# Totoketchup/Adaptive-MultiSpeaker-Separation

Measured on AMD Instinct MI355X. Metric: mixtures/sec training throughput (2-spk, 256-filter adapt+BLSTM-DPCL), higher is better.
Workload: dtype f32 (storage, accumulation and results f32; dense products issued on the 16-bit matrix pipe as fp16x3 / bf16x6 emulation of the f32 product -- `value_native_f32` is the same step on v_mfma_f32_32x32x2_f32)

## Files before the change

### adaptive-multispeaker-separation_amd/ams_hip/functional.py

```python
import torch
from torch.autograd import Function

from . import ops


def _c(t):
    return t if t.is_contiguous() else t.contiguous()


class _Overlap(object):

    def __init__(self):
        self.enabled = False
        self.stream = None
        self.n_cap = 0
        self.deferred = []
        self.on_ready = None

    def side(self):
        if self.stream is None:
            import os
            self.stream = torch.cuda.Stream(priority=int(os.environ.get('AMS_SIDE_PRIORITY', '0')))
        return self.stream

# ... 29 lines not shown
            def __enter__(self_):
                ov.cap(True, kind)

            def __exit__(self_, *exc):
                ov.cap(False)
        return _Cap()

    def ready(self, *params):
        if self.on_ready is not None:
            self.on_ready(params, self.side())

    def defer(self, fn):
        self.deferred.append(fn)

    def flush(self, n=1):
        s = self.side()
        with torch.cuda.stream(s):
            for _ in range(min(n, len(self.deferred))):
                self.deferred.pop(0)()

    def join(self):
        if self.deferred:
            s = self.side()
            s.wait_stream(torch.cuda.current_stream())
            self.flush(len(self.deferred))
        self.n_cap = 0
        if self.stream is not None:
            torch.cuda.current_stream().wait_stream(self.stream)


OVERLAP = _Overlap()


class FrontFilter(Function):

    @staticmethod
    def forward(ctx, w, bases):
        ctx.save_for_backward(w, bases)
        return ops.front_filter(w, bases)

    @staticmethod
    def backward(ctx, df):
        w, bases = ctx.saved_tensors
        return ops.front_filter_bwd(w, bases, _c(df))


class FrontConv(Function):

    @staticmethod
    def forward(ctx, x, f, hop):
        ctx.save_for_backward(x)
        ctx.W, ctx.hop = f.shape[0], hop
        am = (ops.amax_of(x), ops.amax_of(f)) if (ops.F16X3 and x.is_cuda) else None
        return ops.front_conv(x, f, hop, amax=am, measure=True)

    @staticmethod
    def backward(ctx, dy):
        (x,) = ctx.saved_tensors
        df = ops.front_conv_bwd_filter(x, _c(dy), ctx.W, ctx.hop) if ctx.needs_input_grad[1] else None
        return None, df, None


import os as _os
_DW_SPLIT = [int(v) for v in _os.environ.get('AMS_DW_SPLIT', '24,12,4').split(',') if v]


def _dw_cuts(N):
    tiles = N // 256
    if N % 256 or len(_DW_SPLIT) < 2 or tiles < sum(_DW_SPLIT):
        return [(0, N)]
    tot = sum(_DW_SPLIT)
    cuts, n0 = [], 0
    for i, f in enumerate(_DW_SPLIT):
        n1 = N if i == len(_DW_SPLIT) - 1 else n0 + (tiles * f // tot) * 256
        if n1 > n0:
            cuts.append((n0, n1))
        n0 = n1
    return cuts

class BLSTMLayer(Function):

    @staticmethod
    def forward(ctx, x, Kf, bf, Kb, bb, last_capped=False):
        aw = ops.param_amax(Kf) if ops.F16X3 and x.is_cuda else None
        if aw is not None and aw is not ops.param_amax(Kb):
            aw = None
        ax = ops.amax_of(x) if aw is not None else None
        ctx.amax = (ax, aw) if aw is not None else None
        out, G, cst = ops.blstm_fwd(x, Kf, bf, Kb, bb, amax=ctx.amax)
        if x.is_cuda:
            ops.tag_amax(out, ops.amax_one(out.device))
        ctx.last_capped = bool(last_capped)
        ctx.save_for_backward(x, Kf, Kb, out, G, cst)
        ctx.biases = (bf, bb)
        return out

    @staticmethod
    def backward(ctx, dout):
        x, Kf, Kb, out, G, cst = ctx.saved_tensors
        bf, bb = ctx.biases
        need_dx = ctx.needs_input_grad[0]
        if OVERLAP.usable(Kf, Kb, bf, bb) and all(ctx.needs_input_grad[1:5]):
            B, T, D = x.shape
            dbpart = ops.blstm_bwd_recurrent(x, Kf, Kb, G, cst, _c(dout), amax_u=ctx.amax[1] if ctx.amax is not None else None)
            am_dx = am_w = None
            if ctx.amax is not None:
                az = ops.amax_of(G)
                am_dx = (az, ctx.amax[1])
                am_w = (ctx.amax[0], ops.amax_one(G.device), az)
            dx = ops.blstm_bwd_dx(G, Kf, Kb, B, T, D, amax=am_dx) if need_dx else None
            if not need_dx and ops.WGRAD_GROUP >= 1:
                ops.blstm_bwd_weights(x, out, G, Kf.grad, bf.grad, Kb.grad, bb.grad, True, part='all', dbpart=dbpart, amax=am_w)
                return None, None, None, None, None, None
            s = OVERLAP.fork(x, out, G, *([dbpart] if dbpart is not None else []))
            if not need_dx:
                with torch.cuda.stream(s):
                    ops.blstm_bwd_weights(x, out, G, Kf.grad, bf.grad, Kb.grad, bb.grad, True, part='u', amax=am_w)
                ops.blstm_bwd_weights(x, out, G, Kf.grad, bf.grad, Kb.grad, bb.grad, True, part='wx', dbpart=dbpart, amax=am_w)
                return None, None, None, None, None, None
            with torch.cuda.stream(s):
                with OVERLAP.capped('lstm'):
                    ops.blstm_bwd_weights(x, out, G, Kf.grad, bf.grad, Kb.grad, bb.grad, True, part='wx', dbpart=dbpart, amax=am_w)
# ... 10 lines not shown
class BLSTMLayerDropout(Function):

    @staticmethod
    def forward(ctx, x, Kf, bf, Kb, bb, m_in, m_h, m_c, m_out):
        masks = {'in': m_in, 'h': m_h, 'c': m_c, 'out': m_out}
        y, saved = ops.blstm_fwd_dropout(x, Kf, bf, Kb, bb, masks)
        ctx.save_for_backward(x, Kf, Kb, m_in, m_h, m_c, m_out, *saved)
        return y

    @staticmethod
    def backward(ctx, dy):
        x, Kf, Kb, m_in, m_h, m_c, m_out = ctx.saved_tensors[:7]
        saved = ctx.saved_tensors[7:]
        masks = {'in': m_in, 'h': m_h, 'c': m_c, 'out': m_out}
        dx, dKf, dbf, dKb, dbb = ops.blstm_bwd_dropout(_c(dy), x, Kf, Kb, saved, masks, need_dx=ctx.needs_input_grad[0])
        return dx, dKf, dbf, dKb, dbb, None, None, None, None


def blstm_dropout(x, Kf, bf, Kb, bb, keep, masks=None):
    if masks is None:
        B, T, D = x.shape
        masks = ops.blstm_dropout_masks(B, T, D, Kf.shape[1] // 4, keep, x.device)
    return BLSTMLayerDropout.apply(_c(x), Kf, bf, Kb, bb, masks['in'], masks['h'], masks['c'], masks['out'])


class Dense(Function):

    @staticmethod
    def forward(ctx, x, W, b):
        ctx.save_for_backward(x, W)
        ctx.bias = b
        aw = ops.param_amax(W) if ops.F16X3 and x.is_cuda else None
        ctx.amax = (ops.amax_of(x), aw) if aw is not None else None
        return ops.dense_fwd(x, W, b, amax=ctx.amax)

    @staticmethod
    def backward(ctx, du):
        x, W = ctx.saved_tensors
        du2 = _c(du).view(-1, W.shape[1])
        x2 = x.reshape(-1, x.shape[-1])
        b = ctx.bias
        am_dx = am_dw = None
        if ctx.amax is not None:
            adu = ops.amax_of(du2)
            am_dx, am_dw = (adu, ctx.amax[1]), (ctx.amax[0], adu)
        if OVERLAP.usable(W, b) and ctx.needs_input_grad[1] and ctx.needs_input_grad[2]:
            dx = ops.backward_product(du2, W, am_dx, (W,)).view(x.shape) if ctx.needs_input_grad[0] else None
            s = OVERLAP.fork(x2, du2)
            Nw = W.shape[1]
            cuts = _dw_cuts(Nw) if (ctx.needs_input_grad[0] and W.grad.stride(0) == Nw) else [(0, Nw)]

            def piece(n0, n1):
                Wg = W.grad if (n0, n1) == (0, Nw) else W.grad[:, n0:n1]
                dus = du2 if (n0, n1) == (0, Nw) else du2[:, n0:n1]
                with OVERLAP.capped('dense'):
                    fused = ops.gemm_at_b_colsum(x2, dus, Wg, b.grad[n0:n1], accumulate=True, amax=am_dw, ldc=W.grad.stride(0))
                    if not fused:
                        ops.gemm(x2, dus, transA=True, out=Wg, accumulate=True, amax=am_dw, M=x2.shape[1], N=n1 - n0, K=x2.shape[0],
                                 lda=x2.stride(0), ldb=du2.stride(0), ldc=W.grad.stride(0))
                if not fused:
                    ops.colsum_into(_c(dus), b.grad[n0:n1], True)
            with torch.cuda.stream(s):
                piece(*cuts[0])
            for i, c in enumerate(cuts[1:]):
                last = i == len(cuts) - 2
                OVERLAP.defer(lambda c=c, last=last: (piece(*c), OVERLAP.ready(W, b) if last else None))
# ... 766 lines not shown
```

### adaptive-multispeaker-separation_amd/ams_hip/ops.py

```python
import ctypes
import os as _os

import torch

from ._lib import load, check, AmsError

_vp = ctypes.c_void_p


def _p(t):
    return _vp(t.data_ptr()) if t is not None else _vp(0)


def _s():
    return _vp(torch.cuda.current_stream().cuda_stream)


def _chk(*ts):
    for t in ts:
        if t is None:
            continue
        if not t.is_cuda:
            raise AmsError('ams_hip ops need device tensors (there is no CPU fallback)')
        if t.dtype != torch.float32 or not t.is_contiguous():
# ... 664 lines not shown
        raise AmsError('ps_pack_cols: fp32 device matrix with dense rows expected')
    lib = load()
    K, N = w2.shape
    pitch = lib.ams_ps_image_pitch(K)
    if img is None:
        img = torch.empty((N, pitch), dtype=torch.uint8, device=w2.device)
    check(lib.ams_ps_pack_cols(_p(w2), w2.stride(0), _p(img), K, N, _p(amax), _s()), 'ams_ps_pack_cols')
    return img


def gemm_ps(a_img, b_img, K, amax, bias=None, out=None, ldc=None, label=''):
    lib = load()
    M, N = a_img.shape[0], b_img.shape[0]
    if out is None:
        out = torch.empty((M, N), dtype=torch.float32, device=a_img.device)
        ldc = N
    elif ldc is None:
        ldc = out.stride(0) if out.dim() == 2 else N
    ev = PROFILE.begin() if PROFILE.enabled else None
    cur = torch.cuda.current_stream()
    amax[0].record_stream(cur)
    amax[1].record_stream(cur)
    check(lib.ams_gemm_ps(M, N, K, _p(a_img), _p(b_img), _p(out), ldc, _p(bias), _p(amax[0]), _p(amax[1]), _s()), 'ams_gemm_ps')
    PS_LAUNCHES[0] += 1
    if ev is not None:
        PROFILE.end(ev, 2.0 * M * N * K, 4.0 * (M * K + K * N + M * N), 'gemm16ps<0,1>', label)
    return out


def _ps_weight_image(W2, amax_w, owners):
    return derived(owners, 'ps_w', lambda old: (ps_pack_cols(W2, amax_w), amax_w), key=(W2.data_ptr(), W2.shape, id(amax_w)))[0]


def forward_product_presplit(M, N, K, out, bias, amax, label, ldc):
    key = ('gemm', label, M, N, K, False, False)
    return (PRESPLIT and amax is not None and amax[0] is not None and amax[1] is not None and key not in F16_AUDIT.denied
            and not F16_AUDIT.active and LDS_PAD[0] == 0 and N % 4 == 0 and ldc % 4 == 0 and out.data_ptr() % 16 == 0
            and (bias is None or bias.data_ptr() % 16 == 0) and max(M, N) * ((K + 31) // 32 * 128) < 2 ** 31
            and load().ams_gemm_get_arith() != 0)


def forward_product(x2, W2, bias, out, amax, label, owners, ldc=None):
    M, K = x2.shape
    N = W2.shape[1]
    if x2.stride(1) != 1 or W2.stride(1) != 1:
        raise AmsError('forward_product: operands with dense rows expected (strides %r, %r)' % (tuple(x2.stride()), tuple(W2.stride())))
    ldc = (out.stride(0) if out.dim() == 2 else N) if ldc is None else ldc
    if not forward_product_presplit(M, N, K, out, bias, amax, label, ldc):
        return gemm(x2, W2, bias=bias, out=out, M=M, N=N, K=K, lda=x2.stride(0), ldb=W2.stride(0), ldc=ldc, label=label, amax=amax)
    a_img = ps_pack_rows(x2, amax[0])
    b_img = _ps_weight_image(W2, amax[1], owners)
    return gemm_ps(a_img, b_img, K, amax, bias=bias, out=out, ldc=ldc, label=label)


DX_PS = _os.environ.get('AMS_GEMM_DX_PS', '1') != '0'


def _ps_dx_weight_image(W2, amax_w, owners):
    return derived(owners, 'ps_dx', lambda old: (ps_pack_rows(W2, amax_w), amax_w), key=(W2.data_ptr(), W2.shape, id(amax_w)))[0]


def backward_product(dU2, W2, amax, owners, out=None, label=''):
    M, K = dU2.shape
    N = W2.shape[0]
    if out is None:
        out = torch.empty((M, N), dtype=torch.float32, device=dU2.device)
    ldc = out.stride(0) if out.dim() == 2 else N
    lda = dU2.stride(0)
    key = ('gemm', label, M, N, K, False, True)
    lib = load()
    if not (DX_PS and F16X3 and amax is not None and amax[0] is not None and amax[1] is not None and key not in F16_AUDIT.denied
            and not F16_AUDIT.active and LDS_PAD[0] == 0 and N % 4 == 0 and ldc % 4 == 0 and lda % 4 == 0 and dU2.stride(1) == 1
            and W2.stride(1) == 1 and out.data_ptr() % 16 == 0 and dU2.data_ptr() % 16 == 0 and M * lda * 4 < 2 ** 31
            and N * ((K + 31) // 32 * 128) < 2 ** 31 and lib.ams_gemm_get_arith() != 0
            and K % 4 == 0 and (N + 255) // 256 * 256 <= 1.30 * N):
        return gemm(dU2, W2, transB=True, out=out, M=M, N=N, K=K, lda=lda, ldb=W2.stride(0), ldc=ldc, label=label, amax=amax)
    b_img = _ps_dx_weight_image(W2, amax[1], owners)
    nb = lib.ams_gemm_ps_a_workspace_bytes(M, N, K)
    ws = _ws(nb, dU2) if nb else None
    ev = PROFILE.begin() if PROFILE.enabled else None
    cur = torch.cuda.current_stream()
    amax[0].record_stream(cur)
    amax[1].record_stream(cur)
    check(lib.ams_gemm_ps_a_f32(M, N, K, _p(dU2), lda, _p(b_img), _p(out), ldc, _p(amax[0]), _p(amax[1]), _p(ws), nb, _s()),
          'ams_gemm_ps_a_f32')
    if ev is not None:
        PROFILE.end(ev, 2.0 * M * N * K, 4.0 * (M * K + K * N + M * N), 'gemm16ps_a<0,1>', label)
    return out


def gemm_at_b_colsum(A, B, out, bsum, accumulate=True, amax=None, ldc=None):
    K, M = A.shape
    N = B.shape[1]
    ldc = out.stride(0) if ldc is None else ldc
    ok = (M % 4 == 0 and N % 4 == 0 and A.stride(0) % 4 == 0 and B.stride(0) % 4 == 0 and A.stride(1) == 1 and B.stride(1) == 1
          and out.stride(-1) == 1 and bsum.stride(-1) == 1 and not NOVEC)
    if not ok:
        return False
    if any(t.data_ptr() % 16 for t in (A, B, bsum)):
        gemm(A, B, transA=True, out=out, accumulate=accumulate, M=M, N=N, K=K, lda=A.stride(0), ldb=B.stride(0), ldc=ldc, amax=amax,
             key=('at_b_colsum', M, N, K))
        colsum_into(B if B.is_contiguous() else B.contiguous(), bsum, accumulate)
        return True
    lib = load()
    pad = LDS_PAD[0]
    nb = lib.ams_gemm_workspace_bytes(M, N, K, 1, pad)
    ws = _ws(nb, A) if nb else None
    bws = _ws(32 * N * 4, A)
# ... 79 lines not shown
def _err_words():
    live = [r for r in _ERR_EXTRA if r() is not None]
    _ERR_EXTRA[:] = live
    return list(_RING_ERR.values()) + [r() for r in live]


def ring_error_pending():
    return any(bool(t.item() != 0) for t in _err_words())


def ring_errors_clear():
    for t in _err_words():
        t.zero_()


def persist_errors():
    return int(ring_error_pending())


def raise_on_ring_errors():
    if ring_error_pending():
        ring_errors_clear()
        raise AmsError('a BLSTM ring recurrence launch abandoned a bounded wait: its workgroups were not all resident in time '
                       '(another kernel filled the CUs); the results of that step are invalid.  AMS_LSTM_RING=0 selects the '
                       'per-step recurrence kernels, which need no co-residency.')


def _padded_rows(x2, Dp):
    xp = torch.zeros((x2.shape[0], Dp), dtype=x2.dtype, device=x2.device)
    xp[:, :x2.shape[1]].copy_(x2)
    return xp


def blstm_fwd(x, Kf, bf, Kb, bb, amax=None):
    _chk(x, bf, bb)
    _chk_rows(Kf, Kb)
    lib = load()
    B, T, D = x.shape
    H = Kf.shape[1] // 4
    ldu = Kf.stride(0)
    if Kb.stride(0) != ldu:
        raise AmsError('blstm: the two direction kernels must share one row stride')
    x2 = x.view(B * T, D)
    frozen = _frozen(Kf, Kb, bf, bb)
    Wcat = derived((Kf, Kb), 'wcat', lambda old: blstm_wcat(Kf, Kb, D), key=(D,), keep='frozen')
    u_amax = amax[1] if amax is not None else None
    if amax is None and F16X3 and x.is_cuda:
        if frozen:
            u_amax = derived((Kf, Kb), 'kbound', lambda old: torch.maximum(absmax(Kf), absmax(Kb)), keep='frozen')
            amax = (amax_of(x), u_amax)
        else:
            amax = (amax_of(x), derived((Kf, Kb), 'wcat_amax', lambda old: absmax(Wcat, out=old)))
    if _twin(bf, bb):
        bias = torch.as_strided(bf, (8 * H,), (1,))
    else:
        bias = derived((bf, bb), 'bcat', lambda old: torch.cat([bf, bb]), keep='frozen')
    G = torch.empty((B, T, 2, 4 * H), dtype=torch.float32, device=x.device)
    nring = lib.ams_blstm_ring_sync_bytes(B, H, 0) if LSTM_RING != '0' else 0
    out = torch.empty((B, T, 2 * H), dtype=torch.float32, device=x.device)
    cst = torch.empty(((2, B, T, 2, H) if nring else (B, T, 2, H)), dtype=torch.float32, device=x.device)
    blstm_input_projection(x2, Wcat, bias, G.view(B * T, 8 * H), amax, (Kf, Kb))
    if nring:
        sync, pre0 = _ring_sync(nring, x)
        check(lib.ams_blstm_ring_fwd(_p(G), _p(out), _p(cst[0]), _p(cst[1]), _p(Kf[D:]), _p(Kb[D:]), ldu,
                                     _p(u_amax if F16X3 else None), _p(sync), nring, _p(ring_error_word(x.device)), B, T, H,
                                     int(LSTM_RING == 'safe') | pre0, _s()), 'ams_blstm_ring_fwd')
        return out, G, cst
    pack = torch.empty(lib.ams_blstm_pack_floats(H, 0), dtype=torch.float32, device=x.device)
    check(lib.ams_blstm_recurrent_fwd(_p(G), _p(out), _p(cst), _p(Kf[D:]), _p(Kb[D:]), ldu, _p(pack), B, T, H, _s()),
          'ams_blstm_recurrent_fwd')
    return out, G, cst


def blstm_input_projection(x2, Wcat, bias, G2, amax, owners):
    M, D = x2.shape
    N = Wcat.shape[1]
    label = 'blstm_input_gemm'
    Dp = (D + 3) // 4 * 4
    if Dp != D and not forward_product_presplit(M, N, D, G2, bias, amax, label, N):
        Wp = torch.zeros((Dp, N), dtype=Wcat.dtype, device=Wcat.device)
        Wp[:D].copy_(Wcat)
        return gemm(_padded_rows(x2, Dp), Wp, bias=bias, out=G2, M=M, N=N, K=Dp, lda=Dp, ldb=N, ldc=N, label=label, amax=amax,
                    key=('gemm', label, M, N, D, False, False))
    return forward_product(x2, Wcat, bias, G2, amax, label, owners)


def dense_fwd(x, W, b, amax=None):
    x2 = x.reshape(-1, x.shape[-1])
    if x2.stride(1) != 1:
        x2 = x2.contiguous()
    out = torch.empty((x2.shape[0], W.shape[1]), dtype=torch.float32, device=x.device)
    return forward_product(x2, W, b, out, amax, '', (W,)).view(x.shape[:-1] + (W.shape[1],))


def blstm_wcat(Kf, Kb, D):
    H4 = Kf.shape[1]
    if _twin(Kf, Kb):
        return torch.as_strided(Kf, (D, 2 * H4), (2 * H4, 1))
    Wcat = torch.empty((D, 2 * H4), dtype=torch.float32, device=Kf.device)
    Wcat[:, :H4].copy_(Kf[:D])
    Wcat[:, H4:].copy_(Kb[:D])
    return Wcat

# ... 932 lines not shown
```

### adaptive-multispeaker-separation_amd/csrc/gemm_ps.hip

```cpp
#include "common.h"
#include "split.h"
#include <type_traits>

namespace {

typedef __attribute__((address_space(3))) void lds_void;

constexpr int PS_BK = 32, PS_BM = 128, PS_BN = 256, PS_NT = 512;
constexpr int PS_A_BYTES = PS_BM * 128, PS_B_BYTES = PS_BN * 128, PS_STAGE = PS_A_BYTES + PS_B_BYTES;
constexpr int PS_STAGES = 3;
constexpr int PS_BIAS_OFF = PS_STAGES * PS_STAGE;
constexpr int PS_LDS = PS_BIAS_OFF + 2 * 1024;


__global__ __launch_bounds__(256) void ps_pack_rows_kernel(const float* __restrict__ x, long ldx, unsigned char* __restrict__ img,
                                                           unsigned pitch, int R, int K, const float* __restrict__ amax) {
    const int groups = (int)(pitch / 32);
    const long id = (long)blockIdx.x * 256 + threadIdx.x;
    if (id >= (long)R * groups) return;
    const int r = (int)(id / groups), gq = (int)(id - (long)r * groups), k = gq * 8;
    const float s = f16_scale(amax[0]);
    float v[8];
    const float* row = x + (long)r * ldx;
    if (k + 8 <= K && ((((uintptr_t)(row + k)) & 15) == 0)) {
        const float4 a = *reinterpret_cast<const float4*>(row + k), b = *reinterpret_cast<const float4*>(row + k + 4);
        v[0] = a.x; v[1] = a.y; v[2] = a.z; v[3] = a.w; v[4] = b.x; v[5] = b.y; v[6] = b.z; v[7] = b.w;
    } else {
#pragma unroll
        for (int j = 0; j < 8; ++j) v[j] = (k + j < K) ? row[k + j] : 0.f;
    }
    uint4 hi, lo;
    split2h(v[0] * s, v[1] * s, hi.x, lo.x);
    split2h(v[2] * s, v[3] * s, hi.y, lo.y);
    split2h(v[4] * s, v[5] * s, hi.z, lo.z);
    split2h(v[6] * s, v[7] * s, hi.w, lo.w);
    unsigned char* p = img + (long)r * pitch + (k >> 5) * 128 + ((k & 31) >> 3) * 16;
    *reinterpret_cast<uint4*>(p) = hi;
    *reinterpret_cast<uint4*>(p + 64) = lo;
}

constexpr int PS_PC_KT = 4;
__global__ __launch_bounds__(256) void ps_pack_cols_kernel(const float* __restrict__ w, long ldw, unsigned char* __restrict__ img,
                                                           unsigned pitch, int K, int N, const float* __restrict__ amax) {
    __shared__ float t[32][65];
    const int n0 = blockIdx.x * 64;
    const int tx = threadIdx.x & 63, ty = threadIdx.x >> 6;
    const int nl = threadIdx.x >> 2, kg = threadIdx.x & 3;
    const float s = f16_scale(amax[0]);
    const int kt_end = min((int)((K + 31) / 32), (int)(blockIdx.y + 1) * PS_PC_KT);
    float v[8];
    auto fetch = [&](int kt) {
#pragma unroll
        for (int i = 0; i < 8; ++i) {
            const int k = kt * 32 + ty * 8 + i, n = n0 + tx;
            v[i] = (k < K && n < N) ? w[(long)k * ldw + n] : 0.f;
        }
    };
    int kt = blockIdx.y * PS_PC_KT;
    if (kt < kt_end) fetch(kt);
    for (; kt < kt_end; ++kt) {
        __syncthreads();
#pragma unroll
        for (int i = 0; i < 8; ++i) t[ty * 8 + i][tx] = v[i];
        __syncthreads();
        if (kt + 1 < kt_end) fetch(kt + 1);
        if (n0 + nl < N) {
            uint4 hi, lo;
            split2h(t[kg * 8 + 0][nl] * s, t[kg * 8 + 1][nl] * s, hi.x, lo.x);
            split2h(t[kg * 8 + 2][nl] * s, t[kg * 8 + 3][nl] * s, hi.y, lo.y);
            split2h(t[kg * 8 + 4][nl] * s, t[kg * 8 + 5][nl] * s, hi.z, lo.z);
            split2h(t[kg * 8 + 6][nl] * s, t[kg * 8 + 7][nl] * s, hi.w, lo.w);
            unsigned char* p = img + (long)(n0 + nl) * pitch + kt * 128 + kg * 16;
            *reinterpret_cast<uint4*>(p) = hi;
            *reinterpret_cast<uint4*>(p + 64) = lo;
        }
    }
}

__global__ __launch_bounds__(256) void ps_pack_conv_kernel(const float* __restrict__ x, unsigned char* __restrict__ img, int R, int L, int pl,
                                                           unsigned lpp, const float* __restrict__ amax) {
    const long id = (long)blockIdx.x * 256 + threadIdx.x;
    const long per_copy = (long)R * lpp;
    if (id >= 8 * per_copy) return;
    const int c = (int)(id / per_copy);
    const long rem = id - (long)c * per_copy;
    const int sgn = (int)(rem / lpp), t = (int)(rem - (long)sgn * lpp);
    const float s = f16_scale(amax[0]);
    const float* row = x + (long)sgn * L;
    const int i0 = c + 8 * t - pl;
    float v[8];
#pragma unroll
    for (int j = 0; j < 8; ++j) { const int i = i0 + j; v[j] = (i >= 0 && i < L) ? row[i] : 0.f; }
    uint4 hi, lo;
    split2h(v[0] * s, v[1] * s, hi.x, lo.x);
    split2h(v[2] * s, v[3] * s, hi.y, lo.y);
    split2h(v[4] * s, v[5] * s, hi.z, lo.z);
    split2h(v[6] * s, v[7] * s, hi.w, lo.w);
    unsigned char* p = img + (((long)c * R + sgn) * lpp + t) * 32;
    *reinterpret_cast<uint4*>(p) = hi;
    *reinterpret_cast<uint4*>(p + 16) = lo;
}

struct PsArgs {
    const unsigned char* A; const unsigned char* B; float* C; const float* bias;
    const float* amax_a; const float* amax_b;
    int M, N, K;
    long ldc;
// ... 350 lines not shown
            if constexpr (AF32) { setup(wi + 1); start_af32(); }
            else if (nk > 1) issue(1, 1);
        }
    }
}

inline int ps_group_m(int tiles_m, int tiles_n) {
    int gm = 8;
    if (gm > tiles_m) gm = tiles_m;
    (void)tiles_n;
    return gm < 1 ? 1 : gm;
}

}

extern "C" {

size_t ams_ps_image_pitch(int K) { return (size_t)((K + 31) / 32) * 128; }
size_t ams_ps_image_bytes(int rows, int K) { return (size_t)rows * ams_ps_image_pitch(K); }

ams_status ams_ps_pack_rows(const float* x, long ldx, void* img, int R, int K, const float* amax, void* stream) {
    AMS_REQUIRE(x && img && amax && R > 0 && K > 0 && ldx >= K && (((uintptr_t)img) & 15) == 0);
    const unsigned pitch = (unsigned)ams_ps_image_pitch(K);
    const long n = (long)R * (pitch / 32);
    hipLaunchKernelGGL(ps_pack_rows_kernel, dim3((unsigned)((n + 255) / 256)), dim3(256), 0, (hipStream_t)stream, x, ldx, (unsigned char*)img, pitch, R, K, amax);
    return ams_check_launch();
}

ams_status ams_ps_pack_cols(const float* w, long ldw, void* img, int K, int N, const float* amax, void* stream) {
    AMS_REQUIRE(w && img && amax && K > 0 && N > 0 && ldw >= N && (((uintptr_t)img) & 15) == 0);
    const unsigned pitch = (unsigned)ams_ps_image_pitch(K);
    hipLaunchKernelGGL(ps_pack_cols_kernel, dim3((unsigned)((N + 63) / 64), (unsigned)(((K + 31) / 32 + PS_PC_KT - 1) / PS_PC_KT)), dim3(256), 0, (hipStream_t)stream, w, ldw,
                       (unsigned char*)img, pitch, K, N, amax);
    return ams_check_launch();
}

ams_status ams_gemm_ps(int M, int N, int K, const void* A_img, const void* B_img, float* C, long ldc, const float* bias, const float* amax_a,
                       const float* amax_b, void* stream) {
    AMS_REQUIRE(A_img && B_img && C && amax_a && amax_b && M > 0 && N > 0 && K > 0);
    AMS_REQUIRE(N % 4 == 0 && ldc % 4 == 0 && ldc >= N && ((((uintptr_t)C) | ((uintptr_t)bias) | ((uintptr_t)A_img) | ((uintptr_t)B_img)) & 15) == 0);
    PsArgs g{};
    g.A = (const unsigned char*)A_img; g.B = (const unsigned char*)B_img; g.C = C; g.bias = bias; g.amax_a = amax_a; g.amax_b = amax_b;
    g.M = M; g.N = N; g.K = K; g.ldc = ldc;
    g.pitch_a = g.pitch_b = (unsigned)ams_ps_image_pitch(K);
    AMS_REQUIRE((long)M * g.pitch_a < (1L << 31) && (long)N * g.pitch_b < (1L << 31));
    g.tiles_m = (M + PS_BM - 1) / PS_BM; g.tiles_n = (N + PS_BN - 1) / PS_BN;
    g.group_m = ps_group_m(g.tiles_m, g.tiles_n);
    static const int cus = [] { int dev = 0, n = 0; if (hipGetDevice(&dev) != hipSuccess || hipDeviceGetAttribute(&n, hipDeviceAttributeMultiprocessorCount, dev) != hipSuccess || n <= 0) n = 256; return n; }();
    static const bool raised = [] { return hipFuncSetAttribute((const void*)gemm_ps_kernel<false>, hipFuncAttributeMaxDynamicSharedMemorySize, PS_LDS) == hipSuccess; }();
    if (!raised) return AMS_E_LAUNCH_FAILED;
    const int items = g.tiles_m * g.tiles_n;
    int grid = items < cus ? items : cus;
    if (grid >= 8) grid -= grid % 8;
    hipLaunchKernelGGL(gemm_ps_kernel<false>, dim3((unsigned)grid), dim3(PS_NT), PS_LDS, (hipStream_t)stream, g);
    return ams_check_launch();
}

size_t ams_gemm_ps_a_workspace_bytes(int M, int N, int K) {
    if (M <= 0 || N <= 0 || K <= 0) return 0;
    int kps = 0;
    const int splits = ams_detail::dx_splits(M, N, K, ~(size_t)0, &kps);
    return splits > 1 ? (size_t)splits * M * N * sizeof(float) : 0;
}

ams_status ams_gemm_ps_a_f32(int M, int N, int K, const float* A, long lda, const void* B_img, float* C, long ldc, const float* amax_a,
                             const float* amax_b, void* ws, size_t ws_bytes, void* stream) {
// ... 68 lines not shown
```

### adaptive-multispeaker-separation_amd/models/dpcl.py

```python
from ams_hip import functional as F
from ams_hip import ops as K
from ams_hip.graph import Node, get_default_graph, scope
from models.network import Separator
from utils.ops import BLSTM, Conv1D, f_props


class DPCL(Separator):

    def __init__(self, graph=None, **kwargs):
        kwargs['mask_a'] = 1.0
        kwargs['mask_b'] = 0.0

        super(DPCL, self).__init__(graph, **kwargs)
        K.check_dpcl_domain(self.embedding_size, self.S)
        self.init_separator()

    @scope
    def prediction(self):
        self.true_masks = self.y
        self.count_labels_for = self.embedding_size
        E, Fq = self.embedding_size, self.F
        layers = [BLSTM(self.layer_size, name='BLSTM_' + str(i), drop_val=self.rdropout,
                        in_dim=(self.in_dim if i == 0 else self.layer_size)) for i in range(self.nb_layers)]
        conv = Conv1D([1, self.layer_size, E * Fq])
        x_node = self.X

        def _embed(run):
            x = x_node.value(run)
            return conv.f_prop(f_props(layers, x, then=conv))
        self._embed = Node('embed', _embed, register=False)
        self._embed_normalized = True
        return Node('prediction', lambda run: F.l2norm_keep(self._embed.value(run), E)[0], register=False)

    @scope
    def cost(self):
        self.prediction
        embed, y, E = self._embed, self.y, self.embedding_size
        g = get_default_graph()

        def _terms(run):
            u = embed.value(run)
            Y = y.value(run)
            return F.dpcl_loss_u(u, Y.reshape(u.shape[0], -1, Y.shape[-1]), E)
        both = Node('loss', _terms)
        terms = Node('terms', lambda run: both.value(run)[1])
        cost = Node('cost_value', lambda run: both.value(run)[0])
        g.summaries['cost/cost'] = cost
        for k, name in ((1, '1'), (2, '2'), (3, '3')):
            g.summaries['cost/' + name] = Node(name, lambda run, k=k: terms.value(run)[k])
        return cost
```

### adaptive-multispeaker-separation_amd/utils/ops.py

```python
import numpy as np
import torch

from ams_hip import functional as F
from ams_hip.graph import scope, get_scope_variable, get_default_graph

rng = np.random.RandomState(42)


def f_props(layers, x, then=None):
    for i, layer in enumerate(layers):
        if isinstance(layer, BLSTM):
            layer._last_capped = (i == 1 and isinstance(layers[0], BLSTM))
        x = layer.f_prop(x)
    return x


def log10(x):
    return torch.log(x) / np.log(10.0)


def _graph_rng():
    g = get_default_graph()
    if not hasattr(g, '_init_rng'):
        g._init_rng = np.random.RandomState(g.seed)
    return g._init_rng


def xavier_uniform(shape):
    if len(shape) == 1:
        lim = np.sqrt(3.0 / shape[0])
    elif len(shape) == 4:
        rf = shape[0] * shape[1]
        lim = np.sqrt(6.0 / (rf * shape[2] + rf * shape[3]))
    else:
        lim = np.sqrt(6.0 / (shape[0] + shape[1]))
    return _graph_rng().uniform(-lim, lim, size=shape).astype('float32')


def glorot_uniform(shape):
    lim = np.sqrt(6.0 / (shape[0] + shape[1]))
    return _graph_rng().uniform(-lim, lim, size=shape).astype('float32')


class Reshape:
    def __init__(self, shape, name='Reshape'):
        self.shape = shape
# ... 82 lines not shown
```

### include/ams.h

```cpp
#ifndef AMS_H
#define AMS_H
#include <stddef.h>
#include <stdint.h>

#ifdef __cplusplus
extern "C" {
#endif

#define AMS_ABI_VERSION 10

typedef int32_t ams_status;
#define AMS_OK 0
#define AMS_E_INVALID_ARG (-1)
#define AMS_E_WORKSPACE_TOO_SMALL (-2)
#define AMS_E_LAUNCH_FAILED (-3)

int ams_last_error(void);
int ams_abi_version(void);

ams_status ams_front_filter_fwd(const float* w, const float* bases, float* f, int W, int N, void* stream);
ams_status ams_front_filter_bwd(const float* w, const float* bases, const float* df, float* dw, float* dbases, int W, int N,
                                void* stream);

size_t ams_front_conv_fwd_workspace_bytes(int Bt, int L, int W, int N, int hop);
ams_status ams_front_conv_fwd(const float* x, const float* f, float* y, int Bt, int L, int W, int N, int hop, const float* amax_x,
                              const float* amax_f, float* amax_y, int lds_pad, void* ws, size_t ws_bytes, void* sk_scratch,
                              size_t sk_bytes, void* stream);
int ams_front_conv_fwd_measures_output(const float* x, const float* f, int L, int W, int N, int hop);
size_t ams_front_conv_bwd_filter_workspace_bytes(int Bt, int L, int W, int N, int hop);
ams_status ams_front_conv_bwd_filter(const float* x, const float* dy, float* df, int Bt, int L, int W, int N, int hop, void* ws,
                                     size_t ws_bytes, void* stream);

size_t ams_front_maxpool_workspace_bytes(int Bt, int L, int N);
size_t ams_front_maxpool_workspace_bytes_w(int Bt, int L, int N, int W);
ams_status ams_front_maxpool_fwd(const float* x, const float* f, float* y, long long* argmax, int Bt, int L, int W, int N, int P, int hop,
                                 const float* amax_x, const float* amax_f, void* ws, size_t ws_bytes, void* stream);
ams_status ams_argmax_to_pos(const long long* argmax, int32_t* pos, long count, int N, void* stream);
ams_status ams_transpose_f32(const float* in, float* out, int rows, int cols, void* stream);
size_t ams_gather_filter_grad_workspace_bytes(int R, int W, int N);
ams_status ams_gather_filter_grad(const float* x, const float* v, const int32_t* pos, float* df, int R, int L, int W, int N, int T,
                                  int rdiv, void* ws, size_t ws_bytes, void* stream);
ams_status ams_synth_unpool_fwd(const float* vals, const int32_t* pos, const float* f2t, float* out, int R, int L, int W, int N, int T,
                                int P, int hop, int S, void* stream);
ams_status ams_synth_unpool_bwd_vals(const float* dout, const int32_t* pos, const float* f2t, float* dvals, int R, int L, int W, int N,
                                     int T, int S, void* stream);

size_t ams_gemm_workspace_bytes(int M, int N, int K, int nbatch, int lds_pad);
size_t ams_gemm_sk_scratch_bytes(void);
void ams_gemm_set_arith(int mode);
int ams_gemm_get_arith(void);
ams_status ams_gemm_f32(int transA, int transB, int M, int N, int K, const float* A, long lda, const float* B, long ldb, float* C,
                        long ldc, const float* bias, int accumulate, int mask_period, int mask_skip, const float* amax_a,
                        const float* amax_b, int lds_pad, void* ws, size_t ws_bytes, void* sk_scratch, size_t sk_bytes, void* stream);
size_t ams_ps_image_pitch(int K);
size_t ams_ps_image_bytes(int rows, int K);
ams_status ams_ps_pack_rows(const float* x, long ldx, void* img, int R, int K, const float* amax, void* stream);
ams_status ams_ps_pack_cols(const float* w, long ldw, void* img, int K, int N, const float* amax, void* stream);
ams_status ams_gemm_ps(int M, int N, int K, const void* A_img, const void* B_img, float* C, long ldc, const float* bias,
                       const float* amax_a, const float* amax_b, void* stream);
size_t ams_gemm_ps_a_workspace_bytes(int M, int N, int K);
ams_status ams_gemm_ps_a_f32(int M, int N, int K, const float* A, long lda, const void* B_img, float* C, long ldc, const float* amax_a,
                             const float* amax_b, void* ws, size_t ws_bytes, void* stream);

ams_status ams_gemm_f32_at_b_colsum(int M, int N, int K, const float* A, long lda, const float* B, long ldb, float* C, long ldc,
                                    int accumulate, float* bsum_out, int bsum_accumulate, float* bsum_ws, const float* amax_a,
                                    const float* amax_b, int lds_pad, void* ws, size_t ws_bytes, void* sk_scratch, size_t sk_bytes,
                                    void* stream);
size_t ams_blstm_bwd_weights_workspace_bytes(int B, int T, int D, int H, int lds_pad);
ams_status ams_blstm_bwd_weights_f32(int B, int T, int D, int H, const float* x, long ldx, const float* h, const float* dz, float* dK,
                                     long ldk, float* db, int accumulate, const float* bound_x, const float* bound_h, const float* bound_dz,
                                     int lds_pad, void* ws, size_t ws_bytes, void* stream);
size_t ams_dilated_conv2d_workspace_bytes(int B, int T, int F, int cin, int cout, int kh, int kw);
ams_status ams_dilated_conv2d_fwd(const float* x, const float* w, const float* bias, float* y, int B, int T, int F, int cin, int cout,
                                  int kh, int kw, int rt, int rf, const float* amax_x, const float* amax_w, float* amax_y, void* ws,
                                  size_t ws_bytes, void* stream);
ams_status ams_dilated_conv2d_bwd_data(const float* dy, const float* w, const float* y_below, float* dx, int B, int T, int F, int cin,
                                       int cout, int kh, int kw, int rt, int rf, const float* amax_dy, const float* amax_w,
                                       float* amax_dx, void* ws, size_t ws_bytes, void* stream);
ams_status ams_dilated_conv2d_bwd_filter(const float* x, const float* dy, float* dw, float* db, int B, int T, int F, int cin,
                                         int cout, int kh, int kw, int rt, int rf, const float* amax_x, const float* amax_dy, void* ws,
                                         size_t ws_bytes, void* stream);
ams_status ams_dilated_conv2d_relu_bwd(const float* dy, const float* y, float* dx, long n, float* amax_dx, void* stream);
ams_status ams_gemm_f32_batched(int transA, int transB, int M, int N, int K, const float* A, long lda, long a_zs, const float* B,
                                long ldb, long b_zs, float* C, long ldc, long c_zs, int nbatch, int accumulate, int mask_period,
                                int mask_skip, const float* amax_a, const float* amax_b, int lds_pad, void* ws, size_t ws_bytes,
                                void* sk_scratch, size_t sk_bytes, void* stream);
ams_status ams_range_share(const float* x, long rows, long cols, long ld, const float* bound, float* out3, void* stream);
ams_status ams_absmax_f32(const float* x, long n, float* out, void* stream);

ams_status ams_make_masks(const float* rep_non_mix, float* Y, int32_t* argmax, int B, int S, long TF, float a, float b,
// ... 159 lines not shown
```

Measured before the change: 25240.

## Pack downstream weight images on side stream beside BLSTM recurrence

While a BLSTM layer's recurrent kernel runs, the code forks to a side stream and packs the fp16-split weight images for the later BLSTM layers' input projections, the embedding conv and their backward dx products. It also evaluates labels there. A new multi-region pack kernel does all images in one launch and caps its grid at the CUs left idle by the recurrence, with padded LDS to limit occupancy. This hides the pack cost behind the latency-bound recurrence. It adds cross-stream events, record_stream bookkeeping, and possible contention with the recurrent ring kernel.

Result: faster. 25610, median of 6 (+1.4%).

```diff
diff --git a/adaptive-multispeaker-separation_amd/ams_hip/functional.py b/adaptive-multispeaker-separation_amd/ams_hip/functional.py
--- a/adaptive-multispeaker-separation_amd/ams_hip/functional.py
+++ b/adaptive-multispeaker-separation_amd/ams_hip/functional.py
@@ -85,6 +85,77 @@
 OVERLAP = _Overlap()
 
 
+class _ForwardBranch(object):
+
+    def __init__(self):
+        import os
+        self.on = os.environ.get('AMS_FWD_BRANCH', '1') != '0'
+        self.stages = []
+        self.todo = None
+        self.event = None
+        self.fired = self.images = 0
+
+    def arm(self, blstm_params, dense_params, beside=None):
+        self.stages = []
+        if not (self.on and OVERLAP.enabled and torch.is_grad_enabled()):
+            return
+        above = list(blstm_params)
+        self.stages = [(above, None if above else dense_params, beside)]
+        if above and dense_params is not None:
+            self.stages.append(([], dense_params, None))
+
+    def fire(self, x, H, forked):
+        if forked is None:
+            self.todo = self._prepare(x, H)
+            return
+        todo, self.todo = self.todo, None
+        if todo is None:
+            return
+        fwd, dx, beside, wgs, pad = todo
+        main = torch.cuda.current_stream()
+        s = OVERLAP.side()
+        s.wait_event(forked)
+        with torch.cuda.stream(s):
+            self.images += ops.cut_weight_images(fwd, dx, consumer=main, workgroups=wgs, lds_pad=pad)
+            self.fired += 1
+            if beside is not None:
+                for t in beside():
+                    t.record_stream(main)
+            self.event = s.record_event()
+
+    def _prepare(self, x, H):
+        layers, dense, beside = self.stages.pop(0)
+        if not x.is_cuda:
+            return None
+        M = x.shape[0] * x.shape[1]
+        fwd, dx = [], []
+        wgs, pad = ops.beside_ring_launch(x.shape[0], H)
+        for Kf, bf, Kb, bb in (layers if wgs else []):
+            aw = ops.param_amax(Kf) if ops.F16X3 else None
+            if aw is None or aw is not ops.param_amax(Kb) or not ops._twin(Kf, Kb):
+                continue
+            H4 = Kf.shape[1]
+            Wcat = ops.blstm_wcat(Kf, Kb, Kf.shape[0] - H4 // 4)
+            fwd.append((M, Wcat, aw, (Kf, Kb), 'blstm_input_gemm'))
+            if OVERLAP.usable(Kf, Kb, bf, bb):
+                dx.insert(0, (M, Wcat, aw, (Kf, Kb), ''))
+        if dense is not None and wgs:
+            W, b = dense
+            aw = ops.param_amax(W) if ops.F16X3 else None
+            if aw is not None:
+                fwd.append((M, W, aw, (W,), ''))
+                dx.insert(0, (M, W, aw, (W,), ''))
+        return fwd, dx, beside, wgs, pad
+
+    def join(self):
+        ev, self.event = self.event, None
+        if ev is not None:
+            torch.cuda.current_stream().wait_event(ev)
+
+
+FORWARD_BRANCH = _ForwardBranch()
+
+
 class FrontFilter(Function):
 
     @staticmethod
@@ -140,7 +211,9 @@
             aw = None
         ax = ops.amax_of(x) if aw is not None else None
         ctx.amax = (ax, aw) if aw is not None else None
-        out, G, cst = ops.blstm_fwd(x, Kf, bf, Kb, bb, amax=ctx.amax)
+        FORWARD_BRANCH.join()
+        fb = FORWARD_BRANCH
+        out, G, cst = ops.blstm_fwd(x, Kf, bf, Kb, bb, amax=ctx.amax, beside_recurrence=(lambda ev: fb.fire(x, Kf.shape[1] // 4, ev)) if fb.stages else None)
         if x.is_cuda:
             ops.tag_amax(out, ops.amax_one(out.device))
         ctx.last_capped = bool(last_capped)
@@ -217,6 +290,7 @@
         ctx.bias = b
         aw = ops.param_amax(W) if ops.F16X3 and x.is_cuda else None
         ctx.amax = (ops.amax_of(x), aw) if aw is not None else None
+        FORWARD_BRANCH.join()
         return ops.dense_fwd(x, W, b, amax=ctx.amax)
 
     @staticmethod
diff --git a/adaptive-multispeaker-separation_amd/ams_hip/ops.py b/adaptive-multispeaker-separation_amd/ams_hip/ops.py
--- a/adaptive-multispeaker-separation_amd/ams_hip/ops.py
+++ b/adaptive-multispeaker-separation_amd/ams_hip/ops.py
@@ -720,12 +720,16 @@
     return derived(owners, 'ps_w', lambda old: (ps_pack_cols(W2, amax_w), amax_w), key=(W2.data_ptr(), W2.shape, id(amax_w)))[0]
 
 
-def forward_product_presplit(M, N, K, out, bias, amax, label, ldc):
+def _presplit_class(M, N, K, amax, label, ldc):
     key = ('gemm', label, M, N, K, False, False)
     return (PRESPLIT and amax is not None and amax[0] is not None and amax[1] is not None and key not in F16_AUDIT.denied
-            and not F16_AUDIT.active and LDS_PAD[0] == 0 and N % 4 == 0 and ldc % 4 == 0 and out.data_ptr() % 16 == 0
-            and (bias is None or bias.data_ptr() % 16 == 0) and max(M, N) * ((K + 31) // 32 * 128) < 2 ** 31
-            and load().ams_gemm_get_arith() != 0)
+            and not F16_AUDIT.active and LDS_PAD[0] == 0 and N % 4 == 0 and ldc % 4 == 0
+            and max(M, N) * ((K + 31) // 32 * 128) < 2 ** 31 and load().ams_gemm_get_arith() != 0)
+
+
+def forward_product_presplit(M, N, K, out, bias, amax, label, ldc):
+    return (_presplit_class(M, N, K, amax, label, ldc) and out.data_ptr() % 16 == 0
+            and (bias is None or bias.data_ptr() % 16 == 0))
 
 
 def forward_product(x2, W2, bias, out, amax, label, owners, ldc=None):
@@ -748,6 +752,82 @@
     return derived(owners, 'ps_dx', lambda old: (ps_pack_rows(W2, amax_w), amax_w), key=(W2.data_ptr(), W2.shape, id(amax_w)))[0]
 
 
+def _dx_image_class(M, N, K, amax, label):
+    key = ('gemm', label, M, N, K, False, True)
+    return (DX_PS and F16X3 and amax is not None and amax[0] is not None and amax[1] is not None and key not in F16_AUDIT.denied
+            and not F16_AUDIT.active and LDS_PAD[0] == 0 and N % 4 == 0 and N * ((K + 31) // 32 * 128) < 2 ** 31
+            and load().ams_gemm_get_arith() != 0 and K % 4 == 0 and (N + 255) // 256 * 256 <= 1.30 * N)
+
+
+PACK_MANY = _os.environ.get('AMS_PS_PACK_MANY', '1') != '0'
+PS_PACK_MAX = 8
+
+
+class _PackRegion(ctypes.Structure):
+    _fields_ = [('src', ctypes.c_void_p), ('ld', ctypes.c_long), ('img', ctypes.c_void_p), ('amax', ctypes.c_void_p),
+                ('K', ctypes.c_int), ('rows', ctypes.c_int), ('kind', ctypes.c_int), ('pitch', ctypes.c_uint),
+                ('first_block', ctypes.c_uint)]
+
+
+def ps_pack_many(items, imgs=None, workgroups=0, lds_pad=0):
+    lib = load()
+    regs, out = [], []
+    for i, (x2, amax, kind) in enumerate(items):
+        if kind not in ('rows', 'cols'):
+            raise AmsError('ps_pack_many: kind %r' % (kind,))
+        if x2.dtype != torch.float32 or not x2.is_cuda or x2.dim() != 2 or x2.stride(1) != 1:
+            raise AmsError('ps_pack_many: fp32 device matrices with dense rows expected')
+        R, K = x2.shape if kind == 'rows' else (x2.shape[1], x2.shape[0])
+        img = imgs[i] if imgs is not None else torch.empty((R, lib.ams_ps_image_pitch(K)), dtype=torch.uint8, device=x2.device)
+        out.append(img)
+        regs.append(_PackRegion(x2.data_ptr(), x2.stride(0), img.data_ptr(), amax.data_ptr(), K, R, 0 if kind == 'rows' else 1, 0, 0))
+    for i in range(0, len(regs), PS_PACK_MAX):
+        tab = (_PackRegion * len(regs[i:i + PS_PACK_MAX]))(*regs[i:i + PS_PACK_MAX])
+        check(lib.ams_ps_pack_many(ctypes.cast(tab, ctypes.c_void_p), len(tab), int(workgroups), int(lds_pad), _s()), 'ams_ps_pack_many')
+    return out
+
+
+def cut_weight_images(forward, dx, consumer=None, workgroups=0, lds_pad=0):
+    one = None
+    todo = []
+
+    def want(owners, name, W2, amax_w, kind):
+        def make(old):
+            R, K = W2.shape if kind == 'rows' else (W2.shape[1], W2.shape[0])
+            img = torch.empty((R, load().ams_ps_image_pitch(K)), dtype=torch.uint8, device=W2.device)
+            if consumer is not None:
+                img.record_stream(consumer)
+            todo.append(((W2, amax_w, kind), img))
+            return (img, amax_w)
+        derived(owners, name, make, key=(W2.data_ptr(), W2.shape, id(amax_w)))
+
+    for M, W2, amax_w, owners, label in forward:
+        if amax_w is None or not W2.is_cuda or W2.stride(1) != 1:
+            continue
+        one = amax_one(W2.device) if one is None else one
+        K, N = W2.shape
+        if _presplit_class(M, N, K, (one, amax_w), label, N):
+            want(owners, 'ps_w', W2, amax_w, 'cols')
+    for M, W2, amax_w, owners, label in dx:
+        if amax_w is None or not W2.is_cuda or W2.stride(1) != 1:
+            continue
+        one = amax_one(W2.device) if one is None else one
+        N, K = W2.shape
+        if _dx_image_class(M, N, K, (one, amax_w), label):
+            want(owners, 'ps_dx', W2, amax_w, 'rows')
+    if not todo:
+        return 0
+    cur = torch.cuda.current_stream()
+    for (W2, amax_w, kind), img in todo:
+        amax_w.record_stream(cur)
+    if PACK_MANY:
+        ps_pack_many([t[0] for t in todo], imgs=[t[1] for t in todo], workgroups=workgroups, lds_pad=lds_pad)
+    else:
+        for (W2, amax_w, kind), img in todo:
+            (ps_pack_rows if kind == 'rows' else ps_pack_cols)(W2, amax_w, img=img)
+    return len(todo)
+
+
 def backward_product(dU2, W2, amax, owners, out=None, label=''):
     M, K = dU2.shape
     N = W2.shape[0]
@@ -755,13 +835,9 @@
         out = torch.empty((M, N), dtype=torch.float32, device=dU2.device)
     ldc = out.stride(0) if out.dim() == 2 else N
     lda = dU2.stride(0)
-    key = ('gemm', label, M, N, K, False, True)
-    lib = load()
-    if not (DX_PS and F16X3 and amax is not None and amax[0] is not None and amax[1] is not None and key not in F16_AUDIT.denied
-            and not F16_AUDIT.active and LDS_PAD[0] == 0 and N % 4 == 0 and ldc % 4 == 0 and lda % 4 == 0 and dU2.stride(1) == 1
-            and W2.stride(1) == 1 and out.data_ptr() % 16 == 0 and dU2.data_ptr() % 16 == 0 and M * lda * 4 < 2 ** 31
-            and N * ((K + 31) // 32 * 128) < 2 ** 31 and lib.ams_gemm_get_arith() != 0
-            and K % 4 == 0 and (N + 255) // 256 * 256 <= 1.30 * N):
+    lib = load()
+    if not (_dx_image_class(M, N, K, amax, label) and ldc % 4 == 0 and lda % 4 == 0 and dU2.stride(1) == 1
+            and W2.stride(1) == 1 and out.data_ptr() % 16 == 0 and dU2.data_ptr() % 16 == 0 and M * lda * 4 < 2 ** 31):
         return gemm(dU2, W2, transB=True, out=out, M=M, N=N, K=K, lda=lda, ldb=W2.stride(0), ldc=ldc, label=label, amax=amax)
     b_img = _ps_dx_weight_image(W2, amax[1], owners)
     nb = lib.ams_gemm_ps_a_workspace_bytes(M, N, K)
@@ -907,7 +983,16 @@
     return xp
 
 
-def blstm_fwd(x, Kf, bf, Kb, bb, amax=None):
+BESIDE_RING_PAD = 128 * 1024
+
+
+def beside_ring_launch(B, H):
+    cus = torch.cuda.get_device_properties(torch.cuda.current_device()).multi_processor_count
+    idle = cus - 2 * ((B + 15) // 16) * ((H + 11) // 12)
+    return (idle, BESIDE_RING_PAD) if idle >= 8 else (0, 0)
+
+
+def blstm_fwd(x, Kf, bf, Kb, bb, amax=None, beside_recurrence=None):
     _chk(x, bf, bb)
     _chk_rows(Kf, Kb)
     lib = load()
@@ -935,15 +1020,23 @@
     out = torch.empty((B, T, 2 * H), dtype=torch.float32, device=x.device)
     cst = torch.empty(((2, B, T, 2, H) if nring else (B, T, 2, H)), dtype=torch.float32, device=x.device)
     blstm_input_projection(x2, Wcat, bias, G.view(B * T, 8 * H), amax, (Kf, Kb))
+    forked = None
+    if beside_recurrence is not None:
+        beside_recurrence(None)
+        forked = torch.cuda.current_stream().record_event()
     if nring:
         sync, pre0 = _ring_sync(nring, x)
         check(lib.ams_blstm_ring_fwd(_p(G), _p(out), _p(cst[0]), _p(cst[1]), _p(Kf[D:]), _p(Kb[D:]), ldu,
                                      _p(u_amax if F16X3 else None), _p(sync), nring, _p(ring_error_word(x.device)), B, T, H,
                                      int(LSTM_RING == 'safe') | pre0, _s()), 'ams_blstm_ring_fwd')
+        if forked is not None:
+            beside_recurrence(forked)
         return out, G, cst
     pack = torch.empty(lib.ams_blstm_pack_floats(H, 0), dtype=torch.float32, device=x.device)
     check(lib.ams_blstm_recurrent_fwd(_p(G), _p(out), _p(cst), _p(Kf[D:]), _p(Kb[D:]), ldu, _p(pack), B, T, H, _s()),
           'ams_blstm_recurrent_fwd')
+    if forked is not None:
+        beside_recurrence(forked)
     return out, G, cst
 
 
diff --git a/adaptive-multispeaker-separation_amd/csrc/gemm_ps.hip b/adaptive-multispeaker-separation_amd/csrc/gemm_ps.hip
--- a/adaptive-multispeaker-separation_amd/csrc/gemm_ps.hip
+++ b/adaptive-multispeaker-separation_amd/csrc/gemm_ps.hip
@@ -13,10 +13,10 @@
 constexpr int PS_LDS = PS_BIAS_OFF + 2 * 1024;
 
 
-__global__ __launch_bounds__(256) void ps_pack_rows_kernel(const float* __restrict__ x, long ldx, unsigned char* __restrict__ img,
-                                                           unsigned pitch, int R, int K, const float* __restrict__ amax) {
+__device__ __forceinline__ void ps_pack_rows_body(const float* __restrict__ x, long ldx, unsigned char* __restrict__ img,
+                                                  unsigned pitch, int R, int K, const float* __restrict__ amax, unsigned block) {
     const int groups = (int)(pitch / 32);
-    const long id = (long)blockIdx.x * 256 + threadIdx.x;
+    const long id = (long)block * 256 + threadIdx.x;
     if (id >= (long)R * groups) return;
     const int r = (int)(id / groups), gq = (int)(id - (long)r * groups), k = gq * 8;
     const float s = f16_scale(amax[0]);
@@ -39,15 +39,20 @@
     *reinterpret_cast<uint4*>(p + 64) = lo;
 }
 
+__global__ __launch_bounds__(256) void ps_pack_rows_kernel(const float* __restrict__ x, long ldx, unsigned char* __restrict__ img,
+                                                           unsigned pitch, int R, int K, const float* __restrict__ amax) {
+    ps_pack_rows_body(x, ldx, img, pitch, R, K, amax, blockIdx.x);
+}
+
 constexpr int PS_PC_KT = 4;
-__global__ __launch_bounds__(256) void ps_pack_cols_kernel(const float* __restrict__ w, long ldw, unsigned char* __restrict__ img,
-                                                           unsigned pitch, int K, int N, const float* __restrict__ amax) {
+__device__ __forceinline__ void ps_pack_cols_body(const float* __restrict__ w, long ldw, unsigned char* __restrict__ img,
+                                                  unsigned pitch, int K, int N, const float* __restrict__ amax, unsigned bx, unsigned by) {
     __shared__ float t[32][65];
-    const int n0 = blockIdx.x * 64;
+    const int n0 = (int)bx * 64;
     const int tx = threadIdx.x & 63, ty = threadIdx.x >> 6;
     const int nl = threadIdx.x >> 2, kg = threadIdx.x & 3;
     const float s = f16_scale(amax[0]);
-    const int kt_end = min((int)((K + 31) / 32), (int)(blockIdx.y + 1) * PS_PC_KT);
+    const int kt_end = min((int)((K + 31) / 32), (int)(by + 1) * PS_PC_KT);
     float v[8];
     auto fetch = [&](int kt) {
 #pragma unroll
@@ -56,7 +61,7 @@
             v[i] = (k < K && n < N) ? w[(long)k * ldw + n] : 0.f;
         }
     };
-    int kt = blockIdx.y * PS_PC_KT;
+    int kt = (int)by * PS_PC_KT;
     if (kt < kt_end) fetch(kt);
     for (; kt < kt_end; ++kt) {
         __syncthreads();
@@ -73,6 +78,28 @@
             unsigned char* p = img + (long)(n0 + nl) * pitch + kt * 128 + kg * 16;
             *reinterpret_cast<uint4*>(p) = hi;
             *reinterpret_cast<uint4*>(p + 64) = lo;
+        }
+    }
+}
+
+__global__ __launch_bounds__(256) void ps_pack_cols_kernel(const float* __restrict__ w, long ldw, unsigned char* __restrict__ img,
+                                                           unsigned pitch, int K, int N, const float* __restrict__ amax) {
+    ps_pack_cols_body(w, ldw, img, pitch, K, N, amax, blockIdx.x, blockIdx.y);
+}
+
+struct PsPackTable { ams_ps_pack_region r[AMS_PS_PACK_MAX]; int n; unsigned blocks; };
+__global__ __launch_bounds__(256) void ps_pack_many_kernel(const PsPackTable tab) {
+    for (unsigned blk = blockIdx.x; blk < tab.blocks; blk += gridDim.x) {
+        int i = 0;
+#pragma unroll
+        for (int j = 1; j < AMS_PS_PACK_MAX; ++j) i += (j < tab.n && blk >= tab.r[j].first_block) ? 1 : 0;
+        const ams_ps_pack_region& g = tab.r[i];
+        const unsigned local = blk - g.first_block;
+        if (g.kind == AMS_PS_PACK_ROWS) {
+            ps_pack_rows_body(g.src, g.ld, (unsigned char*)g.img, g.pitch, g.rows, g.K, g.amax, local);
+        } else {
+            const unsigned gx = (unsigned)((g.rows + 63) / 64);
+            ps_pack_cols_body(g.src, g.ld, (unsigned char*)g.img, g.pitch, g.K, g.rows, g.amax, local % gx, local / gx);
         }
     }
 }
@@ -489,6 +516,31 @@
     const unsigned pitch = (unsigned)ams_ps_image_pitch(K);
     hipLaunchKernelGGL(ps_pack_cols_kernel, dim3((unsigned)((N + 63) / 64), (unsigned)(((K + 31) / 32 + PS_PC_KT - 1) / PS_PC_KT)), dim3(256), 0, (hipStream_t)stream, w, ldw,
                        (unsigned char*)img, pitch, K, N, amax);
+    return ams_check_launch();
+}
+
+ams_status ams_ps_pack_many(const ams_ps_pack_region* regions, int n, int max_workgroups, int lds_pad, void* stream) {
+    AMS_REQUIRE(regions && n >= 1 && n <= AMS_PS_PACK_MAX && max_workgroups >= 0 && lds_pad >= 0 && lds_pad <= 150 * 1024);
+    PsPackTable tab{};
+    tab.n = n;
+    unsigned long blocks = 0;
+    for (int i = 0; i < n; ++i) {
+        ams_ps_pack_region g = regions[i];
+        AMS_REQUIRE(g.src && g.img && g.amax && g.rows > 0 && g.K > 0 && (((uintptr_t)g.img) & 15) == 0);
+        AMS_REQUIRE(g.kind == AMS_PS_PACK_ROWS || g.kind == AMS_PS_PACK_COLS);
+        AMS_REQUIRE(g.ld >= (g.kind == AMS_PS_PACK_ROWS ? g.K : g.rows));
+        g.pitch = (unsigned)ams_ps_image_pitch(g.K);
+        g.first_block = (unsigned)blocks;
+        if (g.kind == AMS_PS_PACK_ROWS) blocks += (unsigned long)(((long)g.rows * (g.pitch / 32) + 255) / 256);
+        else blocks += (unsigned long)((g.rows + 63) / 64) * (unsigned long)(((g.K + 31) / 32 + PS_PC_KT - 1) / PS_PC_KT);
+        AMS_REQUIRE(blocks < (1UL << 31));
+        tab.r[i] = g;
+    }
+    tab.blocks = (unsigned)blocks;
+    static const bool raised = [] { return hipFuncSetAttribute((const void*)ps_pack_many_kernel, hipFuncAttributeMaxDynamicSharedMemorySize, 150 * 1024) == hipSuccess; }();
+    if (!raised) return AMS_E_LAUNCH_FAILED;
+    const unsigned grid = (max_workgroups > 0 && (unsigned long)max_workgroups < blocks) ? (unsigned)max_workgroups : (unsigned)blocks;
+    hipLaunchKernelGGL(ps_pack_many_kernel, dim3(grid), dim3(256), (size_t)lds_pad, (hipStream_t)stream, tab);
     return ams_check_launch();
 }
 
diff --git a/adaptive-multispeaker-separation_amd/models/dpcl.py b/adaptive-multispeaker-separation_amd/models/dpcl.py
--- a/adaptive-multispeaker-separation_amd/models/dpcl.py
+++ b/adaptive-multispeaker-separation_amd/models/dpcl.py
@@ -25,9 +25,18 @@
         conv = Conv1D([1, self.layer_size, E * Fq])
         x_node = self.X
 
+        def _labels(run):
+            def make():
+                K._DPCL_AHEAD[0] = None
+                y = self.y.value(run)
+                ahead = K._DPCL_AHEAD[0]
+                return [y] + ([ahead[3]] if ahead is not None else [])
+            weighted = self.function_mask in ('linear', 'sqrt', 'square') or self.loss_with_silence
+            return make if (self.plugged and run.training and not weighted and id(self.y) not in run.cache) else None
+
         def _embed(run):
             x = x_node.value(run)
-            return conv.f_prop(f_props(layers, x, then=conv))
+            return conv.f_prop(f_props(layers, x, then=conv, beside=_labels(run)))
         self._embed = Node('embed', _embed, register=False)
         self._embed_normalized = True
         return Node('prediction', lambda run: F.l2norm_keep(self._embed.value(run), E)[0], register=False)
diff --git a/adaptive-multispeaker-separation_amd/utils/ops.py b/adaptive-multispeaker-separation_amd/utils/ops.py
--- a/adaptive-multispeaker-separation_amd/utils/ops.py
+++ b/adaptive-multispeaker-separation_amd/utils/ops.py
@@ -7,11 +7,18 @@
 rng = np.random.RandomState(42)
 
 
-def f_props(layers, x, then=None):
+def f_props(layers, x, then=None, beside=None):
+    from ams_hip.graph import current_run
+    run = current_run()
+    if (run is not None and run.training and layers and all(isinstance(l, BLSTM) and l.drop_val == 0.0 for l in layers)
+            and (then is None or isinstance(then, Conv1D))):
+        F.FORWARD_BRANCH.arm([(l.Kf, l.bf, l.Kb, l.bb) for l in layers[1:]], (then.W, then.b) if then is not None else None, beside)
     for i, layer in enumerate(layers):
         if isinstance(layer, BLSTM):
             layer._last_capped = (i == 1 and isinstance(layers[0], BLSTM))
         x = layer.f_prop(x)
+    F.FORWARD_BRANCH.stages = []
+    F.FORWARD_BRANCH.join()
     return x
 
 
diff --git a/include/ams.h b/include/ams.h
--- a/include/ams.h
+++ b/include/ams.h
@@ -56,6 +56,21 @@
 size_t ams_ps_image_bytes(int rows, int K);
 ams_status ams_ps_pack_rows(const float* x, long ldx, void* img, int R, int K, const float* amax, void* stream);
 ams_status ams_ps_pack_cols(const float* w, long ldw, void* img, int K, int N, const float* amax, void* stream);
+#define AMS_PS_PACK_MAX 8
+#define AMS_PS_PACK_ROWS 0
+#define AMS_PS_PACK_COLS 1
+typedef struct ams_ps_pack_region {
+    const float* src;
+    long ld;
+    void* img;
+    const float* amax;
+    int K;
+    int rows;
+    int kind;
+    unsigned pitch;
+    unsigned first_block;
+} ams_ps_pack_region;
+ams_status ams_ps_pack_many(const ams_ps_pack_region* regions, int n, int max_workgroups, int lds_pad, void* stream);
 ams_status ams_gemm_ps(int M, int N, int K, const void* A_img, const void* B_img, float* C, long ldc, const float* bias,
                        const float* amax_a, const float* amax_b, void* stream);
 size_t ams_gemm_ps_a_workspace_bytes(int M, int N, int K);
```
